# NazirNayal8/RbA

Hardware: AMD Instinct MI355X
Metric: images/sec @1024x2048 Swin-B-1dl (RbA inference hot path) (higher is better)
Workload: dtype f32 (f16x3 split-MFMA GEMMs, fp32 accumulate)

## Files before the change

### rba_amd/csrc/patch_embed.hip

```cpp
#include "common.h"
#include "../../include/rba_hip.h"

namespace {

template <typename T>
__global__ __launch_bounds__(256) void patch_im2col_kernel(const T* __restrict__ img, float* __restrict__ out, int h, int w, int Wt,
                                                          int64_t tokens, float m0, float m1, float m2, float s0, float s1, float s2) {
  const int64_t idx = (int64_t)blockIdx.x * 256 + threadIdx.x;
  const int64_t token = idx >> 4;
  if (token >= tokens) return;
  const int p = (int)(idx & 15);
  f32x4 v = {0.f, 0.f, 0.f, 0.f};
  if (p < 12) {
    const int c = p >> 2, ky = p & 3;
    const int ty = (int)(token / Wt), tx = (int)(token - (int64_t)ty * Wt);
    const int y = 4 * ty + ky, x0 = 4 * tx;
    const float mean = c == 0 ? m0 : (c == 1 ? m1 : m2), sd = c == 0 ? s0 : (c == 1 ? s1 : s2);
    if (y < h) {
      const T* row = img + ((int64_t)c * h + y) * w;
#pragma unroll
      for (int kx = 0; kx < 4; ++kx)
        if (x0 + kx < w) v[kx] = ((float)row[x0 + kx] - mean) / sd;
    }
  }
  *reinterpret_cast<f32x4*>(out + token * 64 + 4 * p) = v;
}

template <typename T>
int launch_im2col(const T* img, float* out, int h, int w, int Hp, int Wp, const float* mean, const float* sd, hipStream_t st) {
  const int Wt = Wp / 4;
  const int64_t tokens = (int64_t)(Hp / 4) * Wt;
  const int64_t threads = tokens * 16;
  hipLaunchKernelGGL(patch_im2col_kernel<T>, dim3((unsigned)((threads + 255) / 256)), dim3(256), 0, st, img, out, h, w, Wt, tokens, mean[0],
                     mean[1], mean[2], sd[0], sd[1], sd[2]);
  return rba_launch_status();
}

}

extern "C" int rba_patch_im2col_u8(const uint8_t* image, float* out, int h, int w, int Hp, int Wp, const float* mean, const float* std,
                                   void* stream) {
  RBA_CHECK_ARG(image && out && mean && std && h >= 1 && w >= 1 && Hp >= h && Wp >= w && (Hp % 4) == 0 && (Wp % 4) == 0);
  RBA_CHECK_ARG(((uintptr_t)out & 15) == 0 && (int64_t)Hp * Wp < (int64_t)1 << 31);
  rba_begin();
  return launch_im2col<uint8_t>(image, out, h, w, Hp, Wp, mean, std, (hipStream_t)stream);
}

extern "C" int rba_patch_im2col_f32(const float* image, float* out, int h, int w, int Hp, int Wp, const float* mean, const float* std,
                                    void* stream) {
  RBA_CHECK_ARG(image && out && mean && std && h >= 1 && w >= 1 && Hp >= h && Wp >= w && (Hp % 4) == 0 && (Wp % 4) == 0);
  RBA_CHECK_ARG(((uintptr_t)out & 15) == 0 && (int64_t)Hp * Wp < (int64_t)1 << 31);
  rba_begin();
  return launch_im2col<float>(image, out, h, w, Hp, Wp, mean, std, (hipStream_t)stream);
}
```

### rba_amd/csrc/resample.hip

```cpp
#include "common.h"
#include "../../include/rba_hip.h"

namespace {

constexpr int CCHUNK = 4;

template <bool ADD, bool VEC4>
__global__ __launch_bounds__(256) void resample_kernel(const float* __restrict__ in, const float* __restrict__ add,
                                                       float* __restrict__ out, int C, int h, int w, int H, int W,
                                                       float sh, float sw, int wq) {
  const int xg = blockIdx.x * blockDim.x + threadIdx.x;
  const int y = blockIdx.y;
  if (xg >= wq) return;
  const int x0 = xg * 4;
  const BilinearTap ty = bilinear_tap(y, sh, h);
  BilinearTap tx[4];
#pragma unroll
  for (int r = 0; r < 4; ++r) tx[r] = bilinear_tap(x0 + r < W ? x0 + r : W - 1, sw, w);
  const int c0 = blockIdx.z * CCHUNK;
  auto one = [&](int c) {
    const float* r0 = in + ((int64_t)c * h + ty.i0) * w;
    const float* r1 = in + ((int64_t)c * h + ty.i1) * w;
    float v[4];
#pragma unroll
    for (int r = 0; r < 4; ++r) {
      const float top = tx[r].l0 * r0[tx[r].i0] + tx[r].l1 * r0[tx[r].i1];
      const float bot = tx[r].l0 * r1[tx[r].i0] + tx[r].l1 * r1[tx[r].i1];
      v[r] = ty.l0 * top + ty.l1 * bot;
    }
    const int64_t o = ((int64_t)c * H + y) * W + x0;
    if (VEC4) {
      f32x4 t = {v[0], v[1], v[2], v[3]};
      if (ADD) {
        t += *reinterpret_cast<const f32x4*>(add + o);
        *reinterpret_cast<f32x4*>(out + o) = t;
      } else {
        __builtin_nontemporal_store(t, reinterpret_cast<f32x4*>(out + o));
      }
    } else {
#pragma unroll
      for (int r = 0; r < 4; ++r)
        if (x0 + r < W) out[o + r] = ADD ? v[r] + add[o + r] : v[r];
    }
  };
  if (c0 + CCHUNK <= C) {
#pragma unroll
    for (int i = 0; i < CCHUNK; ++i) one(c0 + i);
  } else {
    for (int c = c0; c < C; ++c) one(c);
  }
}

struct GnFold {
  const float* mr;
  const float* gamma;
  const float* beta;
  int cpg;
  int relu;
};
__device__ __forceinline__ void gn_fold_coeff(const GnFold& g, int j, f32x4& a, f32x4& b) {
  const int grp = (j << 2) / g.cpg;
  const float mean = g.mr[2 * grp], rstd = g.mr[2 * grp + 1];
  const f32x4 ga = reinterpret_cast<const f32x4*>(g.gamma)[j], be = reinterpret_cast<const f32x4*>(g.beta)[j];
#pragma unroll
  for (int k = 0; k < 4; ++k) {
    a[k] = ga[k] * rstd;
    b[k] = be[k] - mean * a[k];
  }
}
__device__ __forceinline__ f32x4 gn_fold_apply(f32x4 v, const f32x4 a, const f32x4 b, int relu) {
#pragma unroll
  for (int k = 0; k < 4; ++k) {
    v[k] = fmaf(v[k], a[k], b[k]);
    v[k] = rba_clamp_below(v[k], rba_relu_floor(relu));
  }
  return v;
}

template <bool ADD, bool SOUT = false, bool GN = false>
__global__ __launch_bounds__(256) void resample_nhwc_kernel(const float* __restrict__ in, const float* __restrict__ add,
                                                            float* __restrict__ out, int C4, int h, int w, int H, int W, float sh,
                                                            float sw, int64_t row0 = 0, GnFold gin = GnFold{nullptr, nullptr, nullptr, 4, 0},
                                                            GnFold gadd = GnFold{nullptr, nullptr, nullptr, 4, 0}) {
  int64_t idx = (int64_t)blockIdx.x * 256 + threadIdx.x;
  int j;
  int64_t pix;
  if (SOUT) {
    const int64_t wv = idx >> 6;
    const int ln = (int)(idx & 63), nblk = C4 >> 3;
    j = (int)(wv % nblk) * 8 + (ln & 7);
    pix = (wv / nblk) * 8 + (ln >> 3);
    if (pix >= (int64_t)H * W) return;
    idx = pix * C4 + j;
  } else {
    const int64_t total = (int64_t)H * W * C4;
    if (idx >= total) return;
    j = (int)(idx % C4);
    pix = idx / C4;
  }
  const int x = (int)(pix % W), y = (int)(pix / W);
  const BilinearTap ty = bilinear_tap(y, sh, h), tx = bilinear_tap(x, sw, w);
  const f32x4* ip = reinterpret_cast<const f32x4*>(in) + j;
  f32x4 v00 = ip[((int64_t)ty.i0 * w + tx.i0) * C4], v01 = ip[((int64_t)ty.i0 * w + tx.i1) * C4];
  f32x4 v10 = ip[((int64_t)ty.i1 * w + tx.i0) * C4], v11 = ip[((int64_t)ty.i1 * w + tx.i1) * C4];
  if (GN && gin.mr) {
    f32x4 a, b;
    gn_fold_coeff(gin, j, a, b);
    v00 = gn_fold_apply(v00, a, b, gin.relu);
    v01 = gn_fold_apply(v01, a, b, gin.relu);
    v10 = gn_fold_apply(v10, a, b, gin.relu);
    v11 = gn_fold_apply(v11, a, b, gin.relu);
  }
  f32x4 r;
#pragma unroll
  for (int k = 0; k < 4; ++k) {
    const float top = tx.l0 * v00[k] + tx.l1 * v01[k];
    const float bot = tx.l0 * v10[k] + tx.l1 * v11[k];
    r[k] = ty.l0 * top + ty.l1 * bot;
  }
  if (ADD) {
    f32x4 av = reinterpret_cast<const f32x4*>(add)[idx];
    if (GN && gadd.mr) {
      f32x4 a, b;
      gn_fold_coeff(gadd, j, a, b);
      av = gn_fold_apply(av, a, b, gadd.relu);
    }
    r += av;
  }
  if (SOUT) {
    uint32_t hh[2], ll[2];
    rba_split_f16x2(r.x, r.y, hh[0], ll[0]);
    rba_split_f16x2(r.z, r.w, hh[1], ll[1]);
    const bool odd = j & 1;
    const uint32_t s0 = odd ? hh[0] : ll[0], s1 = odd ? hh[1] : ll[1];
    const uint32_t r0 = __builtin_amdgcn_mov_dpp(s0, 0xB1, 0xf, 0xf, true), r1 = __builtin_amdgcn_mov_dpp(s1, 0xB1, 0xf, 0xf, true);
    const rba_u32x4 piece = odd ? (rba_u32x4){r0, r1, ll[0], ll[1]} : (rba_u32x4){hh[0], hh[1], r0, r1};
    const int64_t row = row0 + pix;
    const int k8 = j >> 1;
    const int64_t off = ((row >> 5) * (int64_t)(C4 >> 3) + (k8 >> 2)) * 4096 + ((k8 & 1) * 2 + (odd ? 1 : 0)) * 1024 +
                        (((k8 >> 1) & 1) * 32 + (int)(row & 31)) * 16;
    *reinterpret_cast<rba_u32x4*>(reinterpret_cast<char*>(out) + off) = piece;
  } else {
    reinterpret_cast<f32x4*>(out)[idx] = r;
  }
}

}

extern "C" int rba_resample_bilinear_f32(const float* in, const float* add, float* out, int C, int h, int w, int H, int W,
                                         void* stream) {
  RBA_CHECK_ARG(C >= 0 && h >= 1 && w >= 1 && H >= 0 && W >= 0 && H <= 65535);
  if (C == 0 || H == 0 || W == 0) return 0;
  RBA_CHECK_ARG(in && out);
  const int cz = (C + CCHUNK - 1) / CCHUNK;
  RBA_CHECK_ARG(cz <= 65535);
  rba_begin();
  hipStream_t st = (hipStream_t)stream;
  const int wq = (W + 3) / 4;
  const int threads = wq >= 256 ? 256 : (wq >= 128 ? 128 : 64);
  dim3 grid((wq + threads - 1) / threads, H, cz);
  const float sh = (float)h / (float)H, sw = (float)w / (float)W;
  const bool vec4 = (W % 4 == 0) && ((((uintptr_t)out | (uintptr_t)add) & 15) == 0);
#define RBA_L(A, V) hipLaunchKernelGGL((resample_kernel<A, V>), grid, dim3(threads), 0, st, in, add, out, C, h, w, H, W, sh, sw, wq)
  if (add && vec4) RBA_L(true, true);
  else if (add) RBA_L(true, false);
  else if (vec4) RBA_L(false, true);
  else RBA_L(false, false);
#undef RBA_L
  return rba_launch_status();
}

extern "C" int rba_resample_bilinear_nhwc_f32(const float* in, const float* add, float* out, int C, int h, int w, int H, int W,
                                              void* stream) {
  RBA_CHECK_ARG(C >= 0 && (C & 3) == 0 && h >= 1 && w >= 1 && H >= 0 && W >= 0);
  if (C == 0 || H == 0 || W == 0) return 0;
  RBA_CHECK_ARG(in && out && ((((uintptr_t)in | (uintptr_t)out | (uintptr_t)add) & 15) == 0));
  const int64_t total = (int64_t)H * W * (C >> 2);
  RBA_CHECK_ARG((total + 255) / 256 <= 0x7fffffff);
  rba_begin();
  const float sh = (float)h / (float)H, sw = (float)w / (float)W;
  const dim3 grid((unsigned)((total + 255) / 256));
  if (add)
    hipLaunchKernelGGL(resample_nhwc_kernel<true>, grid, dim3(256), 0, (hipStream_t)stream, in, add, out, C >> 2, h, w, H, W, sh, sw);
  else
    hipLaunchKernelGGL(resample_nhwc_kernel<false>, grid, dim3(256), 0, (hipStream_t)stream, in, add, out, C >> 2, h, w, H, W, sh, sw);
  return rba_launch_status();
}

extern "C" int rba_resample_bilinear_nhwc_split_out_f32(const float* in, const float* add, void* out_frag, int C, int h, int w, int H, int W,
                                                        int64_t row0, void* stream) {
  RBA_CHECK_ARG(C >= 32 && (C % 32) == 0 && h >= 1 && w >= 1 && H >= 0 && W >= 0 && row0 >= 0);
  if (H == 0 || W == 0) return 0;
  RBA_CHECK_ARG(in && out_frag && (((uintptr_t)in | (uintptr_t)add | (uintptr_t)out_frag) & 15) == 0);
  const int64_t total = (((int64_t)H * W + 7) / 8) * 8 * (C >> 2);
  RBA_CHECK_ARG((total + 255) / 256 <= 0x7fffffffLL);
  rba_begin();
  const float sh = (float)h / (float)H, sw = (float)w / (float)W;
  const dim3 grid((unsigned)((total + 255) / 256));
  float* o = reinterpret_cast<float*>(out_frag);
  if (add)
    hipLaunchKernelGGL((resample_nhwc_kernel<true, true>), grid, dim3(256), 0, (hipStream_t)stream, in, add, o, C >> 2, h, w, H, W, sh, sw, row0);
  else
    hipLaunchKernelGGL((resample_nhwc_kernel<false, true>), grid, dim3(256), 0, (hipStream_t)stream, in, add, o, C >> 2, h, w, H, W, sh, sw, row0);
  return rba_launch_status();
}

extern "C" int rba_resample_bilinear_nhwc_gn_f32(const float* in, const float* in_mr, const float* in_gamma, const float* in_beta, int in_relu,
                                                 const float* add, const float* add_mr, const float* add_gamma, const float* add_beta, void* out,
                                                 int split_out, int C, int G, int h, int w, int H, int W, int64_t row0, void* stream) {
  RBA_CHECK_ARG(C >= 4 && (C % 4) == 0 && G >= 1 && (C % G) == 0 && ((C / G) % 4) == 0 && h >= 1 && w >= 1 && H >= 0 && W >= 0 && row0 >= 0);
  RBA_CHECK_ARG(!split_out || (C % 32) == 0);
  if (H == 0 || W == 0) return 0;
  RBA_CHECK_ARG(in && add && out && (!in_mr || (in_gamma && in_beta)) && (!add_mr || (add_gamma && add_beta)));
  RBA_CHECK_ARG((((uintptr_t)in | (uintptr_t)add | (uintptr_t)out | (uintptr_t)in_gamma | (uintptr_t)in_beta | (uintptr_t)add_gamma | (uintptr_t)add_beta) & 15) == 0);
  const int64_t total = split_out ? (((int64_t)H * W + 7) / 8) * 8 * (C >> 2) : (int64_t)H * W * (C >> 2);
  RBA_CHECK_ARG((total + 255) / 256 <= 0x7fffffffLL);
  rba_begin();
  const float sh = (float)h / (float)H, sw = (float)w / (float)W;
  const dim3 grid((unsigned)((total + 255) / 256));
  const GnFold gi{in_mr, in_gamma, in_beta, C / G, in_relu}, ga{add_mr, add_gamma, add_beta, C / G, 0};
  float* o = reinterpret_cast<float*>(out);
  if (split_out)
    hipLaunchKernelGGL((resample_nhwc_kernel<true, true, true>), grid, dim3(256), 0, (hipStream_t)stream, in, add, o, C >> 2, h, w, H, W, sh, sw, row0, gi, ga);
  else
    hipLaunchKernelGGL((resample_nhwc_kernel<true, false, true>), grid, dim3(256), 0, (hipStream_t)stream, in, add, o, C >> 2, h, w, H, W, sh, sw, row0, gi, ga);
  return rba_launch_status();
}
```

Baseline: 154.0.

## Use 2D/3D grids with row-uniform indexing in resample and im2col kernels

Both the patch im2col and the NHWC bilinear resample kernels now map output rows to blockIdx.y/z instead of decoding a flat 64-bit index with divisions. Row taps are made wave-uniform via readfirstlane, offsets use 32-bit arithmetic unless a wide variant is needed, and power-of-two channel counts use shifts. The im2col gains a vectorized 4-wide input load when alignment allows, and GN coefficient loads are hoisted next to the pixel loads. The aim is to cut integer index overhead and improve load issue in these memory-bound kernels, at the cost of more template variants and more complex split-output addressing.

```diff
diff --git a/rba_amd/csrc/patch_embed.hip b/rba_amd/csrc/patch_embed.hip
--- a/rba_amd/csrc/patch_embed.hip
+++ b/rba_amd/csrc/patch_embed.hip
@@ -3,36 +3,48 @@
 
 namespace {
 
-template <typename T>
+template <typename T, bool VEC>
 __global__ __launch_bounds__(256) void patch_im2col_kernel(const T* __restrict__ img, float* __restrict__ out, int h, int w, int Wt,
-                                                          int64_t tokens, float m0, float m1, float m2, float s0, float s1, float s2) {
-  const int64_t idx = (int64_t)blockIdx.x * 256 + threadIdx.x;
-  const int64_t token = idx >> 4;
-  if (token >= tokens) return;
-  const int p = (int)(idx & 15);
+                                                          int Ht, float m0, float m1, float m2, float s0, float s1, float s2) {
+  const int ty = (int)(blockIdx.z * gridDim.y + blockIdx.y);
+  if (ty >= Ht) return;
+  const uint32_t r = blockIdx.x * 256u + threadIdx.x;
+  const int tx = (int)(r >> 4);
+  if (tx >= Wt) return;
+  const int p = (int)(r & 15);
   f32x4 v = {0.f, 0.f, 0.f, 0.f};
   if (p < 12) {
     const int c = p >> 2, ky = p & 3;
-    const int ty = (int)(token / Wt), tx = (int)(token - (int64_t)ty * Wt);
     const int y = 4 * ty + ky, x0 = 4 * tx;
     const float mean = c == 0 ? m0 : (c == 1 ? m1 : m2), sd = c == 0 ? s0 : (c == 1 ? s1 : s2);
     if (y < h) {
-      const T* row = img + ((int64_t)c * h + y) * w;
+      const T* row = img + ((int64_t)(4 * ty) * w + (int64_t)(c * h + ky) * w);
+      if (VEC) {
+        typedef T T4 __attribute__((ext_vector_type(4)));
+        if (x0 < w) {
+          const T4 q = *reinterpret_cast<const T4*>(row + x0);
 #pragma unroll
-      for (int kx = 0; kx < 4; ++kx)
-        if (x0 + kx < w) v[kx] = ((float)row[x0 + kx] - mean) / sd;
+          for (int kx = 0; kx < 4; ++kx) v[kx] = ((float)q[kx] - mean) / sd;
+        }
+      } else {
+#pragma unroll
+        for (int kx = 0; kx < 4; ++kx)
+          if (x0 + kx < w) v[kx] = ((float)row[x0 + kx] - mean) / sd;
+      }
     }
   }
-  *reinterpret_cast<f32x4*>(out + token * 64 + 4 * p) = v;
+  reinterpret_cast<f32x4*>(out + (int64_t)ty * Wt * 64)[r] = v;
 }
 
 template <typename T>
 int launch_im2col(const T* img, float* out, int h, int w, int Hp, int Wp, const float* mean, const float* sd, hipStream_t st) {
   const int Wt = Wp / 4;
-  const int64_t tokens = (int64_t)(Hp / 4) * Wt;
-  const int64_t threads = tokens * 16;
-  hipLaunchKernelGGL(patch_im2col_kernel<T>, dim3((unsigned)((threads + 255) / 256)), dim3(256), 0, st, img, out, h, w, Wt, tokens, mean[0],
-                     mean[1], mean[2], sd[0], sd[1], sd[2]);
+  const int Ht = Hp / 4, gy = Ht < 65535 ? Ht : 65535;
+  const dim3 grid((unsigned)((Wt + 15) / 16), (unsigned)gy, (unsigned)((Ht + gy - 1) / gy));
+  if ((w & 3) == 0 && ((uintptr_t)img & (4 * sizeof(T) - 1)) == 0)
+    hipLaunchKernelGGL((patch_im2col_kernel<T, true>), grid, dim3(256), 0, st, img, out, h, w, Wt, Ht, mean[0], mean[1], mean[2], sd[0], sd[1], sd[2]);
+  else
+    hipLaunchKernelGGL((patch_im2col_kernel<T, false>), grid, dim3(256), 0, st, img, out, h, w, Wt, Ht, mean[0], mean[1], mean[2], sd[0], sd[1], sd[2]);
   return rba_launch_status();
 }
 
diff --git a/rba_amd/csrc/resample.hip b/rba_amd/csrc/resample.hip
--- a/rba_amd/csrc/resample.hip
+++ b/rba_amd/csrc/resample.hip
@@ -1,3 +1,4 @@
+#include <type_traits>
 #include "common.h"
 #include "../../include/rba_hip.h"
 
@@ -57,11 +58,27 @@
   const float* beta;
   int cpg;
   int relu;
+  int qs;
 };
-__device__ __forceinline__ void gn_fold_coeff(const GnFold& g, int j, f32x4& a, f32x4& b) {
-  const int grp = (j << 2) / g.cpg;
-  const float mean = g.mr[2 * grp], rstd = g.mr[2 * grp + 1];
-  const f32x4 ga = reinterpret_cast<const f32x4*>(g.gamma)[j], be = reinterpret_cast<const f32x4*>(g.beta)[j];
+__host__ __device__ inline int rba_log2_exact(int v) {
+  int s = 0;
+  while ((1 << s) < v) ++s;
+  return (1 << s) == v ? s : -1;
+}
+inline GnFold gn_fold(const float* mr, const float* gamma, const float* beta, int cpg, int relu) {
+  return GnFold{mr, gamma, beta, cpg, relu, rba_log2_exact(cpg >> 2)};
+}
+struct GnFoldIn {
+  float mean, rstd;
+  f32x4 ga, be;
+};
+__device__ __forceinline__ GnFoldIn gn_fold_load(const GnFold& g, int j) {
+  const int grp = g.qs >= 0 ? j >> g.qs : (j << 2) / g.cpg;
+  return GnFoldIn{g.mr[2 * grp], g.mr[2 * grp + 1], reinterpret_cast<const f32x4*>(g.gamma)[j], reinterpret_cast<const f32x4*>(g.beta)[j]};
+}
+__device__ __forceinline__ void gn_fold_coeff(const GnFoldIn& in, f32x4& a, f32x4& b) {
+  const float mean = in.mean, rstd = in.rstd;
+  const f32x4 ga = in.ga, be = in.be;
 #pragma unroll
   for (int k = 0; k < 4; ++k) {
     a[k] = ga[k] * rstd;
@@ -77,35 +94,65 @@
   return v;
 }
 
-template <bool ADD, bool SOUT = false, bool GN = false>
+struct ResampleGrid {
+  int c4s;
+  int lognx;
+};
+template <bool ADD, bool SOUT = false, bool GN = false, bool WIDE = false>
 __global__ __launch_bounds__(256) void resample_nhwc_kernel(const float* __restrict__ in, const float* __restrict__ add,
                                                             float* __restrict__ out, int C4, int h, int w, int H, int W, float sh,
-                                                            float sw, int64_t row0 = 0, GnFold gin = GnFold{nullptr, nullptr, nullptr, 4, 0},
-                                                            GnFold gadd = GnFold{nullptr, nullptr, nullptr, 4, 0}) {
-  int64_t idx = (int64_t)blockIdx.x * 256 + threadIdx.x;
-  int j;
-  int64_t pix;
+                                                            float sw, ResampleGrid rg, int64_t row0, GnFold gin, GnFold gadd) {
+  using Off = std::conditional_t<WIDE, int64_t, uint32_t>;
+  const int y = (int)(blockIdx.z * gridDim.y + blockIdx.y);
+  if (y >= H) return;
+  const int wid = __builtin_amdgcn_readfirstlane((int)(threadIdx.x >> 6)), ln = (int)(threadIdx.x & 63);
+  int x, j, x0 = 0, cb = 0;
+  int64_t idx_w;
+  Off idx_l;
   if (SOUT) {
-    const int64_t wv = idx >> 6;
-    const int ln = (int)(idx & 63), nblk = C4 >> 3;
-    j = (int)(wv % nblk) * 8 + (ln & 7);
-    pix = (wv / nblk) * 8 + (ln >> 3);
-    if (pix >= (int64_t)H * W) return;
-    idx = pix * C4 + j;
+    const int nblk = C4 >> 3, bw = nblk < 4 ? nblk : 4;
+    cb = (int)(blockIdx.x & ((1u << rg.lognx) - 1u)) * bw + wid;
+    x0 = (int)(blockIdx.x >> rg.lognx) * 8;
+    if (cb >= nblk) return;
+    x = x0 + (ln >> 3);
+    if (x >= W) return;
+    j = cb * 8 + (ln & 7);
+    idx_w = ((int64_t)y * W + x0) * C4 + cb * 8;
+    idx_l = ((Off)(ln >> 3) * (Off)C4 + (Off)(ln & 7)) * 16;
   } else {
-    const int64_t total = (int64_t)H * W * C4;
-    if (idx >= total) return;
-    j = (int)(idx % C4);
-    pix = idx / C4;
-  }
-  const int x = (int)(pix % W), y = (int)(pix / W);
+    using Row = std::conditional_t<WIDE, int64_t, uint32_t>;
+    const Row r_w = (Row)blockIdx.x * 256 + (Row)(wid * 64);
+    int xw, jw;
+    if (rg.c4s >= 0) {
+      xw = (int)(r_w >> rg.c4s);
+      jw = (int)(r_w & (Row)(C4 - 1));
+    } else {
+      xw = (int)(r_w / (Row)C4);
+      jw = (int)(r_w - (Row)xw * (Row)C4);
+    }
+    const int t = jw + ln, dx = rg.c4s >= 0 ? t >> rg.c4s : (int)((uint32_t)t / (uint32_t)C4);
+    x = xw + dx;
+    if (x >= W) return;
+    j = t - dx * C4;
+    idx_w = (int64_t)y * W * C4 + (int64_t)r_w;
+    idx_l = (Off)ln * 16;
+  }
   const BilinearTap ty = bilinear_tap(y, sh, h), tx = bilinear_tap(x, sw, w);
-  const f32x4* ip = reinterpret_cast<const f32x4*>(in) + j;
-  f32x4 v00 = ip[((int64_t)ty.i0 * w + tx.i0) * C4], v01 = ip[((int64_t)ty.i0 * w + tx.i1) * C4];
-  f32x4 v10 = ip[((int64_t)ty.i1 * w + tx.i0) * C4], v11 = ip[((int64_t)ty.i1 * w + tx.i1) * C4];
+  const int yi0 = __builtin_amdgcn_readfirstlane(ty.i0), yi1 = __builtin_amdgcn_readfirstlane(ty.i1);
+  const char* r0 = reinterpret_cast<const char*>(reinterpret_cast<const f32x4*>(in) + (int64_t)yi0 * w * C4);
+  const char* r1 = reinterpret_cast<const char*>(reinterpret_cast<const f32x4*>(in) + (int64_t)yi1 * w * C4);
+  const Off o0 = ((Off)tx.i0 * (Off)C4 + (Off)j) * 16, o1 = ((Off)tx.i1 * (Off)C4 + (Off)j) * 16;
+  f32x4 v00 = *reinterpret_cast<const f32x4*>(r0 + o0), v01 = *reinterpret_cast<const f32x4*>(r0 + o1);
+  f32x4 v10 = *reinterpret_cast<const f32x4*>(r1 + o0), v11 = *reinterpret_cast<const f32x4*>(r1 + o1);
+  const f32x4 zero4 = {0.f, 0.f, 0.f, 0.f};
+  f32x4 av = zero4;
+  GnFoldIn fin = {0.f, 0.f, zero4, zero4}, fadd = fin;
+  if (ADD) av = *reinterpret_cast<const f32x4*>(reinterpret_cast<const char*>(reinterpret_cast<const f32x4*>(add) + idx_w) + idx_l);
+  if (GN && gin.mr) fin = gn_fold_load(gin, j);
+  if (ADD && GN && gadd.mr) fadd = gn_fold_load(gadd, j);
   if (GN && gin.mr) {
     f32x4 a, b;
-    gn_fold_coeff(gin, j, a, b);
+    gn_fold_coeff(fin, a, b);
     v00 = gn_fold_apply(v00, a, b, gin.relu);
     v01 = gn_fold_apply(v01, a, b, gin.relu);
     v10 = gn_fold_apply(v10, a, b, gin.relu);
@@ -119,10 +166,9 @@
     r[k] = ty.l0 * top + ty.l1 * bot;
   }
   if (ADD) {
-    f32x4 av = reinterpret_cast<const f32x4*>(add)[idx];
     if (GN && gadd.mr) {
       f32x4 a, b;
-      gn_fold_coeff(gadd, j, a, b);
+      gn_fold_coeff(fadd, a, b);
       av = gn_fold_apply(av, a, b, gadd.relu);
     }
     r += av;
@@ -131,18 +177,55 @@
     uint32_t hh[2], ll[2];
     rba_split_f16x2(r.x, r.y, hh[0], ll[0]);
     rba_split_f16x2(r.z, r.w, hh[1], ll[1]);
-    const bool odd = j & 1;
+    const int l7 = ln & 7;
+    const bool odd = l7 & 1;
     const uint32_t s0 = odd ? hh[0] : ll[0], s1 = odd ? hh[1] : ll[1];
     const uint32_t r0 = __builtin_amdgcn_mov_dpp(s0, 0xB1, 0xf, 0xf, true), r1 = __builtin_amdgcn_mov_dpp(s1, 0xB1, 0xf, 0xf, true);
     const rba_u32x4 piece = odd ? (rba_u32x4){r0, r1, ll[0], ll[1]} : (rba_u32x4){hh[0], hh[1], r0, r1};
-    const int64_t row = row0 + pix;
-    const int k8 = j >> 1;
-    const int64_t off = ((row >> 5) * (int64_t)(C4 >> 3) + (k8 >> 2)) * 4096 + ((k8 & 1) * 2 + (odd ? 1 : 0)) * 1024 +
-                        (((k8 >> 1) & 1) * 32 + (int)(row & 31)) * 16;
-    *reinterpret_cast<rba_u32x4*>(reinterpret_cast<char*>(out) + off) = piece;
+    const int64_t row_w = row0 + (int64_t)y * W + x0;
+    const int rl = (int)(row_w & 31) + (ln >> 3);
+    char* ob = reinterpret_cast<char*>(out) + ((row_w >> 5) * (int64_t)(C4 >> 3) + cb) * 4096;
+    const Off off = (Off)(rl >> 5) * (Off)(C4 >> 3) * 4096 + (Off)((((l7 >> 1) & 1) * 2 + (odd ? 1 : 0)) * 1024 + (((l7 >> 2) & 1) * 32 + (rl & 31)) * 16);
+    *reinterpret_cast<rba_u32x4*>(ob + off) = piece;
   } else {
-    reinterpret_cast<f32x4*>(out)[idx] = r;
-  }
+    *reinterpret_cast<f32x4*>(reinterpret_cast<char*>(reinterpret_cast<f32x4*>(out) + idx_w) + idx_l) = r;
+  }
+}
+
+struct ResampleLaunch {
+  dim3 grid, block;
+  ResampleGrid rg;
+  bool wide, ok;
+};
+inline ResampleLaunch resample_nhwc_launch(int C4, int w, int H, int W, bool split_out) {
+  ResampleLaunch L;
+  int64_t gx;
+  L.rg.c4s = rba_log2_exact(C4);
+  L.rg.lognx = 0;
+  if (split_out) {
+    const int nblk = C4 >> 3, bw = nblk < 4 ? nblk : 4, nx = (nblk + bw - 1) / bw;
+    while ((1 << L.rg.lognx) < nx) ++L.rg.lognx;
+    gx = (int64_t)((W + 7) / 8) << L.rg.lognx;
+    L.block = dim3(64 * bw);
+  } else {
+    gx = ((int64_t)W * C4 + 255) / 256;
+    L.block = dim3(256);
+  }
+  const int gy = H < 65535 ? H : 65535;
+  L.ok = gx <= 0x7fffffffLL;
+  L.grid = dim3((unsigned)gx, (unsigned)gy, (unsigned)((H + gy - 1) / gy));
+  const int m = w > W ? w : W;
+  L.wide = (int64_t)(m > 64 ? m : 64) * C4 * 16 > 0xffffffffLL;
+  return L;
+}
+template <bool ADD, bool SOUT, bool GN>
+void resample_nhwc_run(const ResampleLaunch& L, hipStream_t st, const float* in, const float* add, float* out, int C4, int h, int w, int H, int W,
+                       int64_t row0, const GnFold& gi, const GnFold& ga) {
+  const float sh = (float)h / (float)H, sw = (float)w / (float)W;
+  if (L.wide)
+    hipLaunchKernelGGL((resample_nhwc_kernel<ADD, SOUT, GN, true>), L.grid, L.block, 0, st, in, add, out, C4, h, w, H, W, sh, sw, L.rg, row0, gi, ga);
+  else
+    hipLaunchKernelGGL((resample_nhwc_kernel<ADD, SOUT, GN, false>), L.grid, L.block, 0, st, in, add, out, C4, h, w, H, W, sh, sw, L.rg, row0, gi, ga);
 }
 
 }
@@ -176,14 +259,14 @@
   if (C == 0 || H == 0 || W == 0) return 0;
   RBA_CHECK_ARG(in && out && ((((uintptr_t)in | (uintptr_t)out | (uintptr_t)add) & 15) == 0));
   const int64_t total = (int64_t)H * W * (C >> 2);
-  RBA_CHECK_ARG((total + 255) / 256 <= 0x7fffffff);
+  const ResampleLaunch L = resample_nhwc_launch(C >> 2, w, H, W, false);
+  RBA_CHECK_ARG((total + 255) / 256 <= 0x7fffffff && L.ok);
   rba_begin();
-  const float sh = (float)h / (float)H, sw = (float)w / (float)W;
-  const dim3 grid((unsigned)((total + 255) / 256));
+  const GnFold none = gn_fold(nullptr, nullptr, nullptr, 4, 0);
   if (add)
-    hipLaunchKernelGGL(resample_nhwc_kernel<true>, grid, dim3(256), 0, (hipStream_t)stream, in, add, out, C >> 2, h, w, H, W, sh, sw);
+    resample_nhwc_run<true, false, false>(L, (hipStream_t)stream, in, add, out, C >> 2, h, w, H, W, 0, none, none);
   else
-    hipLaunchKernelGGL(resample_nhwc_kernel<false>, grid, dim3(256), 0, (hipStream_t)stream, in, add, out, C >> 2, h, w, H, W, sh, sw);
+    resample_nhwc_run<false, false, false>(L, (hipStream_t)stream, in, add, out, C >> 2, h, w, H, W, 0, none, none);
   return rba_launch_status();
 }
 
@@ -193,15 +276,15 @@
   if (H == 0 || W == 0) return 0;
   RBA_CHECK_ARG(in && out_frag && (((uintptr_t)in | (uintptr_t)add | (uintptr_t)out_frag) & 15) == 0);
   const int64_t total = (((int64_t)H * W + 7) / 8) * 8 * (C >> 2);
-  RBA_CHECK_ARG((total + 255) / 256 <= 0x7fffffffLL);
+  const ResampleLaunch L = resample_nhwc_launch(C >> 2, w, H, W, true);
+  RBA_CHECK_ARG((total + 255) / 256 <= 0x7fffffffLL && L.ok);
   rba_begin();
-  const float sh = (float)h / (float)H, sw = (float)w / (float)W;
-  const dim3 grid((unsigned)((total + 255) / 256));
+  const GnFold none = gn_fold(nullptr, nullptr, nullptr, 4, 0);
   float* o = reinterpret_cast<float*>(out_frag);
   if (add)
-    hipLaunchKernelGGL((resample_nhwc_kernel<true, true>), grid, dim3(256), 0, (hipStream_t)stream, in, add, o, C >> 2, h, w, H, W, sh, sw, row0);
+    resample_nhwc_run<true, true, false>(L, (hipStream_t)stream, in, add, o, C >> 2, h, w, H, W, row0, none, none);
   else
-    hipLaunchKernelGGL((resample_nhwc_kernel<false, true>), grid, dim3(256), 0, (hipStream_t)stream, in, add, o, C >> 2, h, w, H, W, sh, sw, row0);
+    resample_nhwc_run<false, true, false>(L, (hipStream_t)stream, in, add, o, C >> 2, h, w, H, W, row0, none, none);
   return rba_launch_status();
 }
 
@@ -214,15 +297,14 @@
   RBA_CHECK_ARG(in && add && out && (!in_mr || (in_gamma && in_beta)) && (!add_mr || (add_gamma && add_beta)));
   RBA_CHECK_ARG((((uintptr_t)in | (uintptr_t)add | (uintptr_t)out | (uintptr_t)in_gamma | (uintptr_t)in_beta | (uintptr_t)add_gamma | (uintptr_t)add_beta) & 15) == 0);
   const int64_t total = split_out ? (((int64_t)H * W + 7) / 8) * 8 * (C >> 2) : (int64_t)H * W * (C >> 2);
-  RBA_CHECK_ARG((total + 255) / 256 <= 0x7fffffffLL);
+  const ResampleLaunch L = resample_nhwc_launch(C >> 2, w, H, W, split_out != 0);
+  RBA_CHECK_ARG((total + 255) / 256 <= 0x7fffffffLL && L.ok);
   rba_begin();
-  const float sh = (float)h / (float)H, sw = (float)w / (float)W;
-  const dim3 grid((unsigned)((total + 255) / 256));
-  const GnFold gi{in_mr, in_gamma, in_beta, C / G, in_relu}, ga{add_mr, add_gamma, add_beta, C / G, 0};
+  const GnFold gi = gn_fold(in_mr, in_gamma, in_beta, C / G, in_relu), ga = gn_fold(add_mr, add_gamma, add_beta, C / G, 0);
   float* o = reinterpret_cast<float*>(out);
   if (split_out)
-    hipLaunchKernelGGL((resample_nhwc_kernel<true, true, true>), grid, dim3(256), 0, (hipStream_t)stream, in, add, o, C >> 2, h, w, H, W, sh, sw, row0, gi, ga);
+    resample_nhwc_run<true, true, true>(L, (hipStream_t)stream, in, add, o, C >> 2, h, w, H, W, row0, gi, ga);
   else
-    hipLaunchKernelGGL((resample_nhwc_kernel<true, false, true>), grid, dim3(256), 0, (hipStream_t)stream, in, add, o, C >> 2, h, w, H, W, sh, sw, row0, gi, ga);
+    resample_nhwc_run<true, false, true>(L, (hipStream_t)stream, in, add, o, C >> 2, h, w, H, W, row0, gi, ga);
   return rba_launch_status();
 }
```

Result: no change. 154.1 (median of 5 runs) (+0.1%).
